# anrieff/fray

Hardware: AMD Instinct MI355X
Metric: Mrays/s (closest-hit + shadow rays) at 1920x1080, 64spp path trace (higher is better)
Workload: dtype f64

## Files before the change

fray_amd/abi.py:

```python
import ctypes as C

i32, u32, i64, u64, f32, f64 = C.c_int32, C.c_uint32, C.c_int64, C.c_uint64, C.c_float, C.c_double
P = C.POINTER

ABI_VERSION = 3

OK, E_ARG, E_PARSE, E_NODEVICE, E_UNSUPPORTED, E_NOMEM, E_HIP, E_CANCELLED = 0, -1, -2, -3, -4, -5, -6, -7
GEOM_PLANE, GEOM_SPHERE, GEOM_CUBE, GEOM_MESH, GEOM_CSG = range(5)
TEX_CHECKER, TEX_BITMAP, TEX_BUMP, TEX_FRESNEL = range(4)
SHADER_CONST, SHADER_LAMBERT, SHADER_PHONG, SHADER_REFL, SHADER_REFR, SHADER_LAYERED = range(6)
LIGHT_POINT, LIGHT_RECT = range(2)
MODE_PRIMARY_ID, MODE_RENDER = 0, 1
FRAME_STATS = 1
OPTION_NAMES = ("pt_lanes", "pt_budget_mib", "speculate_fans", "fused_whitted_max", "fp_contract", "seed_table_mib", "skip_null_segments",
                "segment_planes", "certified_segments")
FIGURE_NAMES = ("contracted_launches", "shadow_segments", "segment_plane_nodes", "certified_segments_eligible", "shadow_segments_certified",
                "shadow_nodes_skipped", "seed_table_bytes", "seed_launches", "seed_planes_reused", "batch_lanes", "whitted_path",
                "pt_budget_effective_mib", "scene_updates", "scene_update_bytes", "arena_bytes", "fans_filed", "fan_children",
                "fan_children_looked_up", "fans_given_up")


class Transform(C.Structure):
    _fields_ = [("offset", f64 * 3), ("m", f64 * 9), ("invM", f64 * 9)]

# ... 256 lines not shown
    "frayhip_unpack_buckets_device": (C.c_int, [VP, VP, C.c_int, C.c_int, C.c_int, C.c_int, C.c_int, VP]),
    "frayhip_bucket_xy": (C.c_int, [C.c_int, C.c_int, C.c_int, C.POINTER(C.c_int), C.POINTER(C.c_int)]),
    "frayhip_comm_available": (C.c_int, []),
    "frayhip_comm_library": (C.c_char_p, []),
    "frayhip_comm_unique_id": (C.c_int, [VP]),
    "frayhip_comm_create": (C.c_int, [VP, C.c_int, C.c_int, P(VP)]),
    "frayhip_comm_from_nccl": (C.c_int, [VP, C.c_int, C.c_int, P(VP)]),
    "frayhip_comm_ranks": (C.c_int, [VP]),
    "frayhip_comm_destroy": (None, [VP]),
    "frayhip_gather_buckets": (C.c_int, [VP, VP, C.c_int, C.c_int, C.c_int, C.c_int, VP]),
    "frayhip_to_rgb32": (C.c_int, [VP, VP, C.c_int]),
    "frayhip_save_bmp": (C.c_int, [C.c_char_p, VP, C.c_int, C.c_int]),
    "frayhip_debug_rng": (C.c_int, [u32, C.c_int, VP, VP, VP, C.c_int]),
    "frayhip_debug_libm": (C.c_int, [C.c_int, VP, VP, VP, VP, VP]),
    "frayhip_debug_arith": (C.c_int, [C.c_int, C.c_int, VP, VP, VP]),
    "frayhip_last_error": (C.c_char_p, []),
    "frayhip_abi_version": (C.c_int, []),
    "frayhip_sizeof": (C.c_int, [C.c_char_p]),
}


def bind(lib):
    for name, (res, args) in SYMBOLS.items():
        fn = getattr(lib, name)
        fn.restype = res
        fn.argtypes = args
    return lib
```

fray_amd/csrc/capi.hip:

```cpp
#include <hip/hip_runtime.h>

#include <algorithm>
#include <chrono>
#include <cstddef>
#include <cmath>
#include <cstring>
#include <string>
#include <vector>
#include <functional>
#include <cstdlib>


#include "entry_support.hpp"
#include "dev_rng.hpp"
#include "dev_pack.hpp"
#include "scene_arena.hpp"

namespace {

using frayhip_detail::set_error;

void put3(double* o, const double* p) { o[0] = p[0]; o[1] = p[1]; o[2] = p[2]; }
}

// ... 292 lines not shown
    std::vector<frayhip_arena::ArenaMeshTables> meshTables;
    std::vector<int64_t> texelOffset;
    std::vector<unsigned char> host;
    std::vector<int64_t> hostOff;
    int32_t counts[11];
    int64_t nTexels;
    std::vector<frayhip_geom_ref> geoms;
    std::vector<frayhip_csg> csgs;
    std::vector<frayhip_mesh> meshes;
    std::vector<frayhip_texture> textures;
    frayhip_environment environment;
};

namespace frayhip_detail {
const DNode* host_nodes(const frayhip_scene* s) { return (const DNode*)(s->edit->host.data() + s->edit->hostOff[s->edit->F.tNodes]); }
}

namespace {

using frayhip_detail::kStatsBytes;
using frayhip_detail::grid_for;

bool create_lanes(frayhip_scene* sc)
{
    if (hipEventCreateWithFlags(&sc->evLaneStart, hipEventDisableTiming) != hipSuccess) return false;
    for (int k = 0; k < FRAY_PT_LANES; k++) {
        if (k > 0 && hipStreamCreateWithFlags(&sc->laneStream[k], hipStreamNonBlocking) != hipSuccess) return false;
        if (hipEventCreateWithFlags(&sc->evResolved[k], hipEventDisableTiming) != hipSuccess) return false;
    }
    return true;
// ... 211 lines not shown
        set_error("frayhip_scene_create: hipMalloc failed (no device?)");
        delete sc;
        return FRAYHIP_E_NODEVICE;
    }
    {
        unsigned char* const base = (unsigned char*)sc->d_arena;
        std::vector<unsigned char*> stage(B.tables.size());
        std::vector<const unsigned char*> addr(B.tables.size());
        for (size_t t = 0; t < B.tables.size(); t++) { stage[t] = B.host.data() + B.tables[t].off; addr[t] = base + B.tables[t].off; }
        frayhip_arena::arena_place(B.F, B.meshTables.data(), B.texelOffset.data(), stage.data(), addr.data(), sc->S);
    }
    hipError_t e = hipMemcpy(sc->d_arena, B.host.data(), B.host.size(), hipMemcpyHostToDevice);
    if (e != hipSuccess) { set_error(std::string("frayhip_scene_create: upload failed: ") + hipGetErrorString(e)); (void)hipFree(sc->d_arena); delete sc; return FRAYHIP_E_NODEVICE; }
    sc->arena_bytes = B.host.size();
    sc->edit = make_scene_edit(d, B);
    sc->camera = d.camera;
    sc->settings = d.settings;
    if (hipMalloc((void**)&sc->d_stats, kStatsBytes) != hipSuccess || hipMalloc((void**)&sc->d_qmeta, 3 * FRAY_PT_LANES * sizeof(QMeta)) != hipSuccess ||
        hipEventCreate(&sc->evA) != hipSuccess || hipEventCreate(&sc->evB) != hipSuccess || !create_lanes(sc)) {
        set_error("frayhip_scene_create: could not allocate the per-scene device state");
        frayhip_scene_destroy(sc);
        return FRAYHIP_E_NOMEM;
    }
    if (const char* e = getenv("FRAYHIP_PT_LANES")) { long v = atol(e); if (v >= 1 && v <= FRAY_PT_LANES) sc->ptLanes = (int)v; }
    if (const char* e = getenv("FRAYHIP_SPECULATE_FANS")) sc->speculateFans = atol(e) != 0;
    if (const char* e = getenv("FRAYHIP_FP_CONTRACT")) sc->fpContract = atol(e) == 1;
    if (const char* e = getenv("FRAYHIP_SKIP_NULL_SEGMENTS")) sc->skipNullSegments = atol(e) != 0;
    if (const char* e = getenv("FRAYHIP_SEGMENT_PLANES")) sc->segmentPlanes = atol(e) != 0;
    if (const char* e = getenv("FRAYHIP_CERTIFIED_SEGMENTS")) sc->certifiedSegments = atol(e) != 0;
    if (const char* e = getenv("FRAYHIP_FUSED_WHITTED_MAX")) { long v = atol(e); if (v >= 0 && v <= 1024) sc->fusedWhittedMax = (int)v; }
// ... 69 lines not shown
        if (value != 0 && value != 1) { set_error("frayhip_scene_set_option: skip_null_segments must be 0 or 1"); return FRAYHIP_E_ARG; }
        s->skipNullSegments = value != 0;
    } else if (n == "segment_planes") {
        if (value != 0 && value != 1) { set_error("frayhip_scene_set_option: segment_planes must be 0 or 1"); return FRAYHIP_E_ARG; }
        s->segmentPlanes = value != 0;
    } else if (n == "certified_segments") {
        if (value != 0 && value != 1) { set_error("frayhip_scene_set_option: certified_segments must be 0 or 1"); return FRAYHIP_E_ARG; }
        s->certifiedSegments = value != 0;
    } else {
        set_error("frayhip_scene_set_option: unknown option " + n);
        return FRAYHIP_E_ARG;
    }
    return FRAYHIP_OK;
}

int frayhip_scene_set_view(frayhip_scene* s, const frayhip_camera* camera, const frayhip_settings* settings)
{
    if (!s) { set_error("frayhip_scene_set_view: null scene"); return FRAYHIP_E_ARG; }
    if (s->rendering) { set_error("frayhip_scene_set_view: the scene is rendering a frame"); return FRAYHIP_E_ARG; }
    if (settings && (settings->frameWidth <= 0 || settings->frameHeight <= 0)) { set_error("frayhip_scene_set_view: bad frame size"); return FRAYHIP_E_ARG; }
    if (camera) s->camera = *camera;
    if (settings) s->settings = *settings;
    return FRAYHIP_OK;
}

int frayhip_scene_update(frayhip_scene* s, const frayhip_scene_desc* desc)
{
    if (!s || !desc) { set_error("frayhip_scene_update: null argument"); return FRAYHIP_E_ARG; }
    if (s->rendering) { set_error("frayhip_scene_update: the scene is rendering a frame"); return FRAYHIP_E_ARG; }
    if (desc->abi_version != FRAYHIP_ABI_VERSION) { set_error("frayhip_scene_update: ABI version mismatch"); return FRAYHIP_E_ARG; }
// ... 16 lines not shown
        addr[t] = (const unsigned char*)s->d_arena + E.tables[t].off;
    }
    frayhip_arena::arena_update(d, E.meshTables.data(), F, tab.data());
    DScene S = s->S;
    frayhip_arena::arena_place(F, E.meshTables.data(), E.texelOffset.data(), tab.data(), addr.data(), S);
    long long bytes = 0;
    for (int32_t t : frayhip_arena::arena_editable_tables(F)) {
        if (!E.tables[t].bytes) continue;
        HIP_TRY(hipMemcpy((unsigned char*)s->d_arena + E.tables[t].off, tab[t], E.tables[t].bytes, hipMemcpyHostToDevice));
        bytes += (long long)E.tables[t].bytes;
    }
    E.host.swap(next);
    E.F = F;
    commit_facts(s, F);
    s->S = S;
    s->sceneUpdates++;
    s->sceneUpdateBytes = bytes;
    return FRAYHIP_OK;
}

void frayhip_scene_destroy(frayhip_scene* s)
{
    if (!s) return;
    delete s->edit;
    if (s->d_arena) (void)hipFree(s->d_arena);
    if (s->d_work) (void)hipFree(s->d_work);
    frayhip_detail::seed_table_free(s);
    if (s->d_stats) (void)hipFree(s->d_stats);
    if (s->d_motionTab) (void)hipFree(s->d_motionTab);
    if (s->d_qmeta) (void)hipFree(s->d_qmeta);
    if (s->evA) (void)hipEventDestroy(s->evA);
    if (s->evB) (void)hipEventDestroy(s->evB);
    if (s->evLaneStart) (void)hipEventDestroy(s->evLaneStart);
    for (int k = 0; k < FRAY_PT_LANES; k++) {
        if (s->evResolved[k]) (void)hipEventDestroy(s->evResolved[k]);
        if (s->laneStream[k]) (void)hipStreamDestroy(s->laneStream[k]);
    }
    for (auto e : s->evPool) (void)hipEventDestroy(e);
    for (auto e : s->evPoolShadow) (void)hipEventDestroy(e);
    delete s;
}
// ... 164 lines not shown
```

fray_amd/csrc/dev_trace.hpp:

```cpp
#pragma once
#ifndef FRAY_IDENTITY_SKIP
#define FRAY_IDENTITY_SKIP 1
#endif
#ifndef FRAY_FILTER_STRAIGHT
#define FRAY_FILTER_STRAIGHT 1
#endif
#include "dev_math.hpp"
#include "dev_scene.hpp"
#include "dev_sort.hpp"
#define FRAY_CERT_SEQ() __builtin_amdgcn_sched_barrier(0)
#include "dev_boxcert.hpp"
#include "dev_misscert.hpp"
#include "dev_segcert.hpp"

#ifdef FRAY_LEAFSTAT
static __device__ unsigned long long g_leafStat[4];
#endif
struct Cnt {
    unsigned long long closest, shadow, node, kdInner, leafRefs, tri, prim, smooth, samples, tex;
    unsigned envelope;
};
template <int ST> FD void bump(unsigned long long& c, unsigned long long n = 1) { if (ST & 1) c += n; }
constexpr bool kd_variant(int st) { return (st & 6) != 0; }
constexpr bool tex_variant(int st) { return (st & 14) != 0; }
// ... 110 lines not shown
        best = gamma;
        l2o = l2;
        l3o = l3;
    }
    return hit;
}

FD void tri_bary(const FRAY_RO DTri* T, V3 s, V3 d, double& l2, double& l3)
{
    const V3 N = ld3(T->N), A = ld3(T->A), AC = ld3(T->AC), AB = ld3(T->AB);
    const V3 D = -d;
    const double rDcr = fray_rcp(dot(N, D));
    const V3 H = s - A;
    l2 = dot(cross(H, AC), D) * rDcr;
    l3 = dot(cross(AB, H), D) * rDcr;
}

FD V3 ray_rdir(V3 d)
{
    V3 rd;
    rd.x = fabs(d.x) > 1e-12 ? fray_rcp(d.x) : 1e12;
    rd.y = fabs(d.y) > 1e-12 ? fray_rcp(d.y) : 1e12;
    rd.z = fabs(d.z) > 1e-12 ? fray_rcp(d.z) : 1e12;
    return rd;
}
template <int ST>
FD void prepare_ray(LocalRay& lr)
{
    if (lr.haveRd) return;
    lr.rd = ray_rdir(lr.d);
// ... 736 lines not shown
        const FRAY_RO DNode& W = S.nodes[best.node];
        if (W.geomKind == 3 && S.meshes[W.geomIndex].smooth) c.smooth++;
    }
    STAMP(6);
    const int nl = S.nLights;
    for (int i = 0; i < nl; i++) {
        double dist;
        if (light_intersect<ST>(S.lights[i], o, d, dist, c) && dist < best.dist) {
            best.node = -2 - i;
            best.dist = dist;
        }
    }
    STAMP(7);
}

FD uint32_t segment_skip_nodes(const DScene& S, V3 a, V3 b, bool live)
{
    const int nP = S.segmentPlanes ? S.nSegPlanes : 0;
    if (nP <= 0) return 0u;
    const V3 e = b - a;
    const double m = seg_cert_scale(a.x, a.y, a.z, b.x, b.y, b.z, e.x, e.y, e.z);
    const lanes_t all = lanes(true);
    uint32_t certified = 0;
    for (int p = 0; p < nP; p++) {
        const FRAY_RO DSegPlane& P = S.segPlanes[p];
        if (lanes(!live || seg_same_side(P.N[0], P.N[1], P.N[2], P.k, P.t0, P.t1, m, a.x, a.y, a.z, b.x, b.y, b.z)) == all) certified |= 1u << p;
    }
    uint32_t skipNodes = 0;
    const int nS = S.nSegNodes;
    for (int j = 0; j < nS; j++)
// ... 77 lines not shown
```

fray_amd/csrc/kernels.hpp:

```cpp
#pragma once
#include "dev_shade.hpp"
#include "dev_whitted.hpp"
#include "dev_queues.hpp"
#include <type_traits>

#ifndef FRAY_PRIMARY_WAVES
#define FRAY_PRIMARY_WAVES 5
#endif
#ifndef FRAY_WHITTED_WAVES
#define FRAY_WHITTED_WAVES 3
#endif
#ifndef FRAY_WHITTED_REFILL
#define FRAY_WHITTED_REFILL 64
#endif
#ifndef FRAY_CSG_WAVES
#define FRAY_CSG_WAVES 3
#endif
constexpr int waves_for(int st, int n) { return (st & 2) ? (FRAY_CSG_WAVES < n ? FRAY_CSG_WAVES : n) : ((st & 1) && n > 2 ? n - 1 : n); }
#ifndef FRAY_MT_EARLY
#define FRAY_MT_EARLY 160
#endif
#ifndef FRAY_WH_SHADE_WAVES
#define FRAY_WH_SHADE_WAVES 4
#endif
// ... 959 lines not shown
        spawn_ray(sh, info, win, ps.tab, wout, brdf, pdf);
        {
            ps.pm = ps.pm * brdf / pdf;
            ps.o = wout.o; ps.d = wout.d; ps.depth = wout.depth; ps.flags = wout.flags;
#ifdef FRAY_SORT_BY_MATERIAL
            ps.flags = (ps.flags & 0xffu) | ((sh.kind == 1 ? 0u : sh.kind == 3 ? 1u : sh.kind == 4 ? 2u : 3u) << 8);
#endif
            if (ps.depth > S.maxTraceDepth || intensity(ps.pm) < 0.01) path_finish(TB, st, ps, SB);
            else cont = true;
        }
    }
    if (!shadow) term_store(TB, ps.slot, own);
}

struct LongRng { uint32_t* cols; uint32_t nPaths; DFrame F; int nItems, s0; };
struct FirstArgs { DCamera C; DFrame F; int nItems, s0; uint32_t n; const uint32_t* x397; unsigned short* termCount; };
struct BounceArgs { DScene S; PathQueue Qin, Qout; ShadowQueue SQ; QMetaRO metaIn; QMeta* metaOut; QMeta* metaShadow; TermBuf TB; StereoBuf SB; LongRng LR; DStats* st; FirstArgs FA; unsigned long long* segCertified; };
#ifndef FRAY_ARITH
#define FRAY_ARITH 0
#endif
template <int ST, bool LONG, bool FIRST = false, int ARITH = FRAY_ARITH>
static __global__ __launch_bounds__(256, waves_for(ST, kd_variant(ST) ? FRAY_BOUNCE_WAVES : FRAY_BOUNCE_WAVES_NOKD)) void k_pt_bounce(BounceArgs A)
{
    static_assert(!(LONG && FIRST), "long generators start from k_pt_init");
    typedef typename std::conditional<LONG, MtPath, Mt>::type G;
    Cnt c = zero_cnt();
    const QMetaRO metaIn = A.metaIn;
    QMeta* const metaOut = A.metaOut;
    QMeta* const metaShadow = A.metaShadow;
    DStats* const st = A.st;
    const FRAY_RO uint32_t* off = FIRST ? nullptr : metaIn.p->off;
    const FRAY_RO uint32_t* nfIn = FIRST ? nullptr : metaIn.p->nf;
    const uint32_t nSeg = FIRST ? 1u : metaIn.p->nSeg, chunkIn = FIRST ? A.FA.n : metaIn.p->chunk;
    const bool certFront = !FIRST && metaIn.p->certFront != 0;
    const WaveShare ws = wave_share(FIRST ? A.FA.n : metaIn.p->n);
    const uint32_t lane = threadIdx.x & 63u;
    SegEnds outEnds{ws.begin, ws.chunk, 0, 0};
    __shared__ uint32_t shadowCount[4][ST == 0 ? 3 : 2];
    if (lane < (ST == 0 ? 3u : 2u)) shadowCount[threadIdx.x >> 6][lane] = 0;
// ... 44 lines not shown
                }
            }
        } else {
            if constexpr (SORT) i = live ? sorted[di - b0] : 0u;
            else i = seg_map(off, nfIn, nSeg, chunkIn, base, di, live, seg);
            gateFree = certFront && (i & FRAY_FRONT_BIT);
            i &= ~FRAY_FRONT_BIT;
            if (live) {
                path_load_ray(Qin, i, ps);
                live = !(ps.d.x == 0 && ps.d.y == 0 && ps.d.z == 0);
            }
        }
        if (live) {
            STAMP(0);
            HitT<ST> h;
            closest_hit<ST>(S, ps.o, ps.d, h, c, gateFree);
            if constexpr (FIRST) {
                ps.pm = c3(1, 1, 1); ps.slot = di; ps.depth = 0; ps.flags = 0;
                ps.rnd = mt_seed_with(seed0, FA.x397[di]);
                ps.tab = ps.rnd;
                mt_skip(ps.rnd, 2);
                if (FA.C.dof) mt_skip(ps.tab, 4);
                bump<ST>(c.samples);
            } else {
                path_load_rest(Qin, i, ps);
            }
#ifdef FRAY_QCHECK
            if (ps.slot >= TB.nPaths) { atomicAdd(&st->rngOverflow, 1ull << 32); ps.slot = 0; ps.pm = c3(0, 0, 0); ps.depth = 0x7fff; }
            else Qin.rec[i].slot = 0xffffffffu;
#endif
            if constexpr (LONG) {
// ... 27 lines not shown
    if (lane == 0) {
        metaOut->cnt[ws.w] = outEnds.nF + outEnds.nB; metaOut->nf[ws.w] = outEnds.nF;
        metaShadow->cnt[ws.w] = shadowCount[threadIdx.x >> 6][0] + shadowCount[threadIdx.x >> 6][1]; metaShadow->nf[ws.w] = shadowCount[threadIdx.x >> 6][0];
        if constexpr (ST == 0) {
            unsigned long long* const total = KARG(BounceArgs, kernel_args<BounceArgs>(), segCertified);
            const uint32_t nCert = shadowCount[threadIdx.x >> 6][2];
            if (total && nCert) atomicAdd(total, (unsigned long long)nCert);
        }
    }
    if (blockIdx.x == 0 && threadIdx.x == 0) {
        metaOut->chunk = ws.chunk; metaOut->nSeg = ws.W; metaShadow->chunk = ws.chunk; metaShadow->nSeg = ws.W;
        metaOut->certFront = metaShadow->certFront = A.S.gatesExact ? 1u : 0u;
    }
    if (ST & 1) flush_stats(st, c);
    if ((ST & 2) && c.envelope) atomicAdd(&st->rngOverflow, 1ull);
}

struct ShadowArgs { DScene S; ShadowQueue SQ; QMetaRO meta; TermBuf TB; DStats* st; unsigned long long* segSkipped; };
template <int ST, int ARITH = FRAY_ARITH>
static __global__ __launch_bounds__(256, anyhit_waves(ST)) void k_pt_shadow(ShadowArgs A)
{
    Cnt c = zero_cnt();
    const QMetaRO meta = A.meta;
    DStats* const st = A.st;
    const FRAY_RO uint32_t* off = meta.p->off;
    const FRAY_RO uint32_t* nfIn = meta.p->nf;
    const uint32_t nSeg = meta.p->nSeg, chunkIn = meta.p->chunk;
    const bool certFront = meta.p->certFront != 0;
    const WaveShare ws = wave_share(meta.p->n);
    const uint32_t lane = threadIdx.x & 63u;
// ... 177 lines not shown
```

fray_amd/csrc/render_impl.hpp:

```cpp
#pragma once
#include <algorithm>
#include <chrono>
#include <cstring>
#include <cstdio>

#include "accum.hpp"
#include "entry_support.hpp"
#include "kernels.hpp"

namespace frayhip_detail {

namespace {
unsigned char* carve_queue(unsigned char* p, size_t n, PathQueue& Q)
{
    Carve c{p};
    Q.rec = (PathRec*)c.take(n * sizeof(PathRec));
    Q.cls = c.take(n);
    return c.p;
}
size_t queue_bytes(size_t n) { return r256(n * sizeof(PathRec)) + r256(n); }
unsigned char* carve_shadow(unsigned char* p, size_t n, ShadowQueue& Q)
{
    Carve c{p};
    Q.ax = (double*)c.take(n * 8); Q.ay = (double*)c.take(n * 8); Q.az = (double*)c.take(n * 8);
// ... 167 lines not shown
    Batches B;
    B.sc = sc; B.prog = prog; B.t0 = t0; B.F = F; B.nItems = nItems; B.d_rgb = d_rgb;
    B.frameBytes = (size_t)W * H * 12;
    B.acc = acc; B.first = first;
    B.total = B.samplesDone = f->mode == FRAYHIP_MODE_PRIMARY_ID ? 1 : first + spp;

    struct Drain { frayhip_scene* sc; bool armed = true; ~Drain() { if (armed) { (void)hipDeviceSynchronize(); seed_table_invalidate(sc); } } } drain{sc};
    sc->seedTab.serving = false;
    sc->lastSeedLaunches = sc->lastSeedReused = 0;
    sc->lastBatchLanes = 1;
    HIP_TRY(hipMemsetAsync(sc->d_stats, 0, kStatsBytes, stream));
    DCursors* cursors = (DCursors*)((unsigned char*)sc->d_stats + kCursorOffset);
    HIP_TRY(hipEventRecord(sc->evA, stream));
    size_t nTraceEvents = 0, nShadowEvents = 0;
    long long nContracted = 0;
    const unsigned long long* fanTotals = nullptr;

    if (f->mode == FRAYHIP_MODE_PRIMARY_ID) {
        if (nItems > 0) {
            hipEvent_t a = pool_event(sc->evPool, 0), b = pool_event(sc->evPool, 1);
            HIP_TRY(hipEventRecord(a, stream));
            hipLaunchKernelGGL(k_primary<ST>, dim3(persistent_grid(nItems, primary_waves(ST))), dim3(256), 0, stream, PrimaryArgs{S, C, F, nItems, d_id, d_dist, sc->d_stats, cursors});
            HIP_TRY(hipEventRecord(b, stream));
            nTraceEvents = 2;
        }
    } else if (f->mode == FRAYHIP_MODE_RENDER) {
        if (!d_rgb && !acc) { set_error("frayhip_render: MODE_RENDER needs an rgb buffer"); return FRAYHIP_E_ARG; }
        if (set.maxTraceDepth < 0) {
            if (nItems > 0 && acc) launch_acc_black(grid_for(nItems), stream, F, nItems, first, spp, sc->camera.stereoSeparation > 0 ? 2 : 1, acc->accum, sc->d_stats);
            else if (nItems > 0) hipLaunchKernelGGL(k_black, dim3(grid_for(nItems)), dim3(256), 0, stream, F, nItems, sc->camera.stereoSeparation > 0 ? 2 : 1, d_rgb, sc->d_stats);
// ... 188 lines not shown
            if (maxLanes > 1 && !(sc->warmMask & warmKey) && !getenv("FRAYHIP_NO_PRIME")) {
                HIP_TRY(hipMemsetAsync(sc->d_qmeta, 0, 3 * FRAY_PT_LANES * sizeof(QMeta), stream));
                HIP_TRY(hipStreamSynchronize(stream));
                for (int k = 0; k < maxLanes; k++) {
                    hipStream_t ws = k == 0 ? stream : sc->laneStream[k];
                    QMeta* m = sc->d_qmeta + 3 * k;
                    const QMetaRO mIn{(const FRAY_RO QMeta*)m};
                    BounceArgs BA{};
                    BA.S = S; BA.metaIn = mIn; BA.metaOut = m + 1; BA.metaShadow = m + 2; BA.st = sc->d_stats;
                    ShadowArgs SA{};
                    SA.S = S; SA.meta = mIn; SA.st = sc->d_stats + 1;
                    if (longRngW) hipLaunchKernelGGL((k_pt_bounce<ST, true>), dim3(1), dim3(256), 0, ws, BA);
                    else {
                        hipLaunchKernelGGL((k_pt_bounce<ST, false>), dim3(1), dim3(256), 0, ws, BA);
                        hipLaunchKernelGGL((k_pt_bounce<ST, false, true>), dim3(1), dim3(256), 0, ws, BA);
                    }
                    hipLaunchKernelGGL(k_pt_shadow<ST>, dim3(1), dim3(256), 0, ws, SA);
                    if constexpr (!(ST & 2)) {
                        if (sc->fpContract) { launch_bounce_contracted<ST>(1, ws, BA); launch_shadow_contracted<ST>(1, ws, SA); }
                    }
                    HIP_TRY(hipStreamSynchronize(ws));
                }
                sc->warmMask |= warmKey;
            }
            if (maxLanes > 3 && (size_t)nItems * (size_t)spp < ((size_t)24 << 20)) maxLanes = 3;
            const bool stereo = sc->camera.stereoSeparation > 0;
            int chunk = 0, nBatches = 0, nLanes = 0;
            size_t nPaths = 0, nQueue = 0, laneBytes = 0;
            if (first == 0) seed_table_begin(sc, F, nItems, spp);
            for (;;) {
// ... 48 lines not shown
                if (!sc->seedTab.serving) { L.seedWords = (uint32_t*)p; p += (nPaths * 4 + 255) / 256 * 256; }
                L.terms = (float*)p; p += (nPaths * (size_t)(set.maxTraceDepth + 2) * 12 + 255) / 256 * 256;
                L.termCount = (unsigned short*)p; p += (nPaths * 2 + 255) / 256 * 256;
                L.mtCols = nullptr;
                if (longRng) { L.mtCols = (uint32_t*)p; p += (nPaths * 2 * 624 * sizeof(uint32_t) + 255) / 256 * 256; }
                L.SB = StereoBuf{};
                L.sampleRadR = nullptr;
                if (stereo) {
                    L.sampleRadR = (float*)p; p += (nPaths * 12 + 255) / 256 * 256;
                    for (int q = 0; q < 6; q++) { L.SB.r[q] = (double*)p; p += (nPaths * 8 + 255) / 256 * 256; }
                    for (int q = 0; q < 6; q++) { L.SB.g[q] = (uint32_t*)p; p += (nPaths * 4 + 255) / 256 * 256; }
                }
            }
            const StereoBuf SBnone{};
            const int nBounce = set.maxTraceDepth + 2;
            HIP_TRY(hipEventRecord(sc->evLaneStart, stream));
            for (int k = 1; k < nLanes; k++) HIP_TRY(hipStreamWaitEvent(sc->laneStream[k], sc->evLaneStart, 0));
            auto trace = [&](int batch) -> int {
                const int s0 = first + batch * chunk, cn = std::min(chunk, spp - batch * chunk);
                Lane& L = lane[batch % nLanes];
                hipStream_t ls = L.stream;
                const uint32_t* x397 = nullptr;
                if (const int rc = seed_batch(sc, F, nItems, s0, cn, L.seedWords, ls, x397)) return rc;
                for (int eye = 0; eye < (stereo ? 2 : 1); eye++) {
                    const bool fused = !stereo && !longRng;
                    float* rad = eye == 0 ? L.sampleRad : L.sampleRadR;
                    const StereoBuf& save = (stereo && eye == 0) ? L.SB : SBnone;
                    if (!fused) {
                        hipLaunchKernelGGL(k_meta_dense, dim3(1), dim3(64), 0, ls, L.meta, (uint32_t)((size_t)nItems * cn));
                        hipLaunchKernelGGL(k_pt_init<ST>, dim3(grid_for((size_t)nItems * cn)), dim3(256), 0, ls, S, C, F, nItems, s0, cn, L.Q[0],
                                           L.termCount, x397, L.SB, eye, sc->d_stats);
                    }
                    for (int b = 0; b < nBounce; b++) {
                        const QMetaRO mIn{(const FRAY_RO QMeta*)(L.meta + (b & 1))}, mSh{(const FRAY_RO QMeta*)(L.meta + 2)};
                        const int grid = bounce_grid((size_t)nItems * cn, (ST & 2) != 0 && nLanes == 1);
                        hipEvent_t ea = pool_event(sc->evPool, nTraceEvents), eb = pool_event(sc->evPool, nTraceEvents + 1);
                        hipEvent_t ec = pool_event(sc->evPoolShadow, nShadowEvents), ed = pool_event(sc->evPoolShadow, nShadowEvents + 1);
                        if (!ea || !eb || !ec || !ed) return FRAYHIP_E_NOMEM;
                        HIP_TRY(hipEventRecord(ea, ls));
                        const LongRng LR{L.mtCols, (uint32_t)nPaths, F, nItems, s0};
                        const TermBuf TB{L.terms, L.termCount, (uint32_t)nPaths, b};
                        const FirstArgs FA{C, F, nItems, s0, (uint32_t)((size_t)nItems * cn), x397, L.termCount};
                        const BounceArgs BA{S, L.Q[b & 1], L.Q[(b + 1) & 1], L.SQ, mIn, L.meta + ((b + 1) & 1), L.meta + 2, TB, save, LR, sc->d_stats, FA, L.segCertified};
                        bool contractedLaunch = false;
                        if constexpr (!(ST & 2)) {
                            if (sc->fpContract && !longRng && b > 0) { launch_bounce_contracted<ST>(grid, ls, BA); contractedLaunch = true; nContracted++; }
                        }
                        if (contractedLaunch) {}
                        else if (longRng) hipLaunchKernelGGL((k_pt_bounce<ST, true>), dim3(grid), dim3(256), 0, ls, BA);
                        else if (fused && b == 0) hipLaunchKernelGGL((k_pt_bounce<ST, false, true>), dim3(grid), dim3(256), 0, ls, BA);
                        else hipLaunchKernelGGL((k_pt_bounce<ST, false>), dim3(grid), dim3(256), 0, ls, BA);
                        HIP_TRY(hipEventRecord(eb, ls));
                        nTraceEvents += 2;
                        hipLaunchKernelGGL(k_scan, dim3(2), dim3(1024), 0, ls, L.meta + ((b + 1) & 1), L.meta + 2, L.segTotal);
                        HIP_TRY(hipEventRecord(ec, ls));
                        bool contractedShadow = false;
                        if constexpr (!(ST & 2)) {
                            if (sc->fpContract) { launch_shadow_contracted<ST>(grid, ls, ShadowArgs{S, L.SQ, mSh, TB, sc->d_stats + 1, L.segSkipped}); contractedShadow = true; nContracted++; }
                        }
                        if (!contractedShadow) hipLaunchKernelGGL(k_pt_shadow<ST>, dim3(grid), dim3(256), 0, ls, ShadowArgs{S, L.SQ, mSh, TB, sc->d_stats + 1, L.segSkipped});
                        HIP_TRY(hipEventRecord(ed, ls));
                        nShadowEvents += 2;
                    }
                    if (stereo) hipLaunchKernelGGL(k_pt_fold, dim3(grid_for((size_t)nItems * cn)), dim3(256), 0, ls, TermBuf{L.terms, L.termCount, (uint32_t)nPaths, 0},
// ... 31 lines not shown
                  "the shadow-queue totals, the skipped nodes and the certified segments follow the counter blocks");
    HIP_TRY(hipMemcpy(&back, sc->d_stats, sizeof back, hipMemcpyDeviceToHost));
    const DStats (&dsv)[2] = back.ds;
    sc->lastShadowSegments = 0;
    for (int k = 0; k < FRAY_PT_LANES; k++) sc->lastShadowSegments += (long long)back.segTotal[k];
    sc->lastShadowCertified = 0;
    for (int k = 0; k < FRAY_PT_LANES; k++) sc->lastShadowCertified += (long long)back.segCertified[k];
    sc->lastShadowSegments += sc->lastShadowCertified;
    sc->lastShadowNodesSkipped = 0;
    for (int k = 0; k < FRAY_PT_LANES; k++) sc->lastShadowNodesSkipped += (long long)back.segSkipped[k];
    {
        unsigned long long ft[4] = {0, 0, 0, 0};
        if (fanTotals) HIP_TRY(hipMemcpy(ft, fanTotals, sizeof ft, hipMemcpyDeviceToHost));
        for (int q = 0; q < 4; q++) sc->lastFans[q] = (long long)ft[q];
        sc->lastContracted = nContracted;
    }
#ifdef FRAY_LEAFSTAT
    {
        unsigned long long ls[4] = {0, 0, 0, 0}, zero[4] = {0, 0, 0, 0};
        (void)hipMemcpyFromSymbol(ls, HIP_SYMBOL(g_leafStat), sizeof ls);
        (void)hipMemcpyToSymbol(HIP_SYMBOL(g_leafStat), zero, sizeof zero);
        if (ls[0]) fprintf(stderr, "[leafstat] wave leaf phases %llu, all active lanes in ONE leaf %.1f %%, active lanes per phase %.1f, distinct leaves per phase %.2f\n",
                           ls[0], 100.0 * (double)ls[1] / (double)ls[0], (double)ls[2] / (double)ls[0], (double)ls[3] / (double)ls[0]);
    }
#endif
#ifdef FRAY_TILESTAT
    if (const char* out = getenv("FRAY_TILESTAT_OUT")) {
        std::vector<unsigned long long> ts(65536 * 8);
        (void)hipMemcpyFromSymbol(ts.data(), HIP_SYMBOL(g_tileStat), ts.size() * sizeof(unsigned long long));
        if (FILE* fp = fopen(out, "wb")) { fwrite(ts.data(), sizeof(unsigned long long), ts.size(), fp); fclose(fp); }
// ... 51 lines not shown
```

fray_amd/csrc/render_state.hpp:

```cpp
#pragma once
#include <hip/hip_runtime.h>

#include <cstddef>
#include <string>
#include <vector>

#include "capi_common.h"
#include "dev_scene.hpp"
#include "dev_queues.hpp"

namespace frayhip_detail {
inline int hip_error_code(hipError_t e)
{
    switch (e) {
        case hipErrorOutOfMemory: return FRAYHIP_E_NOMEM;
        case hipErrorNoDevice: case hipErrorInvalidDevice: case hipErrorInsufficientDriver: case hipErrorNotInitialized: return FRAYHIP_E_NODEVICE;
        default: return FRAYHIP_E_HIP;
    }
}
}
#define HIP_TRY(expr)                                                                             \
    do {                                                                                          \
        hipError_t e_ = (expr);                                                                   \
        if (e_ != hipSuccess) {                                                                   \
// ... 35 lines not shown
    frayhip_camera camera{};
    frayhip_settings settings{};
    bool whittedNeedsRecursion = false;
    int specFanMax = 0;
    bool speculateFans = true;
    bool lightDraws = false;
    int lastWhittedPath = 0;
    int fusedWhittedMax = 4;
    int csgLanes = 1;
    unsigned warmMask = 0;
    bool fpContract = false;
    long long lastContracted = 0;
    bool skipNullSegments = true;
    bool segmentPlanes = true;
    bool certifiedSegments = true;
    long long lastShadowCertified = 0;
    long long lastShadowNodesSkipped = 0;
    long long lastShadowSegments = 0;
    long long lastFans[4] = {0, 0, 0, 0};
    int lightSampleCount = 0;
    bool extGeometry = false;
    bool textured = false;
    bool kdMeshes = false;
    void* d_work = nullptr;
    size_t work_bytes = 0;
    DStats* d_stats = nullptr;
    void* d_motionTab = nullptr;
    size_t motionTabBytes = 0;
    std::vector<unsigned char> motionTabHost;
    QMeta* d_qmeta = nullptr;
// ... 43 lines not shown
```

fray_amd/scene.py:

```python
import ctypes as C
import math
import os
import sys

import numpy as np

from . import abi

P = C.POINTER

_HERE = os.path.dirname(os.path.abspath(__file__))
_LIB_PATH = os.environ.get("FRAYHIP_LIB") or os.path.join(_HERE, "libfrayhip.so")


class FrayError(RuntimeError):
    def __init__(self, code, msg):
        super().__init__("frayhip error %d: %s" % (code, msg))
        self.code = code


def _load():
    if "torch" not in sys.modules and not os.environ.get("FRAYHIP_NO_TORCH"):
        try:
            import torch
# ... 545 lines not shown
    def endRender(self):
        if self._dev:
            lib.frayhip_scene_destroy(self._dev)
            self._dev = C.c_void_p()

    def set_option(self, name, value):
        self._need_dev()
        _check(lib.frayhip_scene_set_option(self._dev, name.encode(), int(value)))
        return self

    def get_option(self, name):
        self._need_dev()
        v = C.c_int64(0)
        _check(lib.frayhip_scene_get_option(self._dev, name.encode(), C.byref(v)))
        return int(v.value)

    def _frame(self, mode, seed, bucket_first, bucket_stride, spp_chunk, stats):
        return abi.Frame(mode=mode, seed=seed, bucket_first=bucket_first, bucket_stride=bucket_stride,
                         spp_chunk=spp_chunk, flags=abi.FRAME_STATS if stats else 0)

    def _need_dev(self):
        if not self._dev:
            raise FrayError(abi.E_ARG, "Scene.beginRender() has not been called")

    def render(self, seed=42, bucket_first=0, bucket_stride=1, spp_chunk=0, stats=False, out=None, progress=None, preview_ms=-1):
        self._need_dev()
        W, H = self.frame_size
        rgb = out if out is not None else np.zeros((H, W, 3), np.float32)
        st = abi.Stats()
        fr = self._frame(abi.MODE_RENDER, seed, bucket_first, bucket_stride, spp_chunk, stats)
# ... 514 lines not shown
```

include/frayhip.h:

```cpp
#ifndef FRAYHIP_H
#define FRAYHIP_H

#include <stdint.h>

#ifdef __cplusplus
extern "C" {
#endif

#define FRAYHIP_ABI_VERSION 3

enum {
    FRAYHIP_OK            = 0,
    FRAYHIP_E_ARG         = -1,
    FRAYHIP_E_PARSE       = -2,
    FRAYHIP_E_NODEVICE    = -3,
    FRAYHIP_E_UNSUPPORTED = -4,
    FRAYHIP_E_NOMEM       = -5,
    FRAYHIP_E_HIP         = -6,
    FRAYHIP_E_CANCELLED   = -7,
};


typedef struct frayhip_transform {
    double offset[3];
// ... 397 lines not shown
int  frayhip_comm_unique_id(void* id128);
int  frayhip_comm_create(const void* id128, int rank, int world, frayhip_comm** out);
int  frayhip_comm_from_nccl(void* nccl_comm, int rank, int world, frayhip_comm** out);
int  frayhip_comm_ranks(frayhip_comm* c);
void frayhip_comm_destroy(frayhip_comm* c);
int  frayhip_gather_buckets(frayhip_comm* c, float* d_frame, int width, int height, int channels, int root, void* hip_stream);

int  frayhip_to_rgb32(const float* rgb, uint32_t* out, int n_pixels);

int  frayhip_save_bmp(const char* path, const float* rgb, int width, int height);

int  frayhip_debug_rng(uint32_t seed, int n, float* floats, double* doubles, int32_t* ints, int int_hi);

int  frayhip_debug_libm(int n, const double* x, double* sin_out, double* cos_out, double* acos_out, double* acos_arg);

int  frayhip_debug_arith(int op, int n, const double* a, const double* b, double* out);

const char* frayhip_last_error(void);
int  frayhip_abi_version(void);
int  frayhip_sizeof(const char* struct_name);

#ifdef __cplusplus
}
#endif
#endif
```

Baseline: 13290.

## Precompute per-frame camera-origin table for first-bounce triangle tests

Adds a per-frame kernel that, for the camera position, precomputes each node's local-space origin and per-triangle origin-dependent terms (N·H, H×AC, AB×H). The fused first-bounce kernel then uses a specialised closest-hit that reads these values instead of recomputing the transform and cross products per ray. This cuts arithmetic for primary rays in exchange for extra memory traffic, a small single-block setup kernel, and a device buffer sized by the triangle count. It is enabled by default for the plain stats-free path and skipped for stereo, depth of field and long RNG.

```diff
diff --git a/fray_amd/abi.py b/fray_amd/abi.py
--- a/fray_amd/abi.py
+++ b/fray_amd/abi.py
@@ -294,6 +294,7 @@
     "frayhip_debug_rng": (C.c_int, [u32, C.c_int, VP, VP, VP, C.c_int]),
     "frayhip_debug_libm": (C.c_int, [C.c_int, VP, VP, VP, VP, VP]),
     "frayhip_debug_arith": (C.c_int, [C.c_int, C.c_int, VP, VP, VP]),
+    "frayhip_debug_camera_table": (C.c_int, [VP, P(C.c_int64)]),
     "frayhip_last_error": (C.c_char_p, []),
     "frayhip_abi_version": (C.c_int, []),
     "frayhip_sizeof": (C.c_int, [C.c_char_p]),
diff --git a/fray_amd/csrc/capi.hip b/fray_amd/csrc/capi.hip
--- a/fray_amd/csrc/capi.hip
+++ b/fray_amd/csrc/capi.hip
@@ -330,6 +330,13 @@
 
 namespace frayhip_detail {
 const DNode* host_nodes(const frayhip_scene* s) { return (const DNode*)(s->edit->host.data() + s->edit->hostOff[s->edit->F.tNodes]); }
+int count_tl_tris(const frayhip_scene* s)
+{
+    const DNode* nodes = host_nodes(s);
+    long long n = 0;
+    for (int i = 0; i < s->edit->F.nNodes; i++) n += nodes[i].tlTris;
+    return (int)std::min<long long>(n, 0x7fffffff);
+}
 }
 
 namespace {
@@ -571,6 +578,7 @@
     if (e != hipSuccess) { set_error(std::string("frayhip_scene_create: upload failed: ") + hipGetErrorString(e)); (void)hipFree(sc->d_arena); delete sc; return FRAYHIP_E_NODEVICE; }
     sc->arena_bytes = B.host.size();
     sc->edit = make_scene_edit(d, B);
+    sc->camTabTris = frayhip_detail::count_tl_tris(sc);
     sc->camera = d.camera;
     sc->settings = d.settings;
     if (hipMalloc((void**)&sc->d_stats, kStatsBytes) != hipSuccess || hipMalloc((void**)&sc->d_qmeta, 3 * FRAY_PT_LANES * sizeof(QMeta)) != hipSuccess ||
@@ -670,6 +678,13 @@
     return FRAYHIP_OK;
 }
 
+int frayhip_debug_camera_table(frayhip_scene* s, int64_t* used)
+{
+    if (!s || !used) { set_error("frayhip_debug_camera_table: null argument"); return FRAYHIP_E_ARG; }
+    *used = s->lastCameraTable ? 1 : 0;
+    return FRAYHIP_OK;
+}
+
 int frayhip_scene_set_view(frayhip_scene* s, const frayhip_camera* camera, const frayhip_settings* settings)
 {
     if (!s) { set_error("frayhip_scene_set_view: null scene"); return FRAYHIP_E_ARG; }
@@ -716,6 +731,7 @@
     E.F = F;
     commit_facts(s, F);
     s->S = S;
+    s->camTabTris = frayhip_detail::count_tl_tris(s);
     s->sceneUpdates++;
     s->sceneUpdateBytes = bytes;
     return FRAYHIP_OK;
@@ -727,6 +743,7 @@
     delete s->edit;
     if (s->d_arena) (void)hipFree(s->d_arena);
     if (s->d_work) (void)hipFree(s->d_work);
+    if (s->d_camTab) (void)hipFree(s->d_camTab);
     frayhip_detail::seed_table_free(s);
     if (s->d_stats) (void)hipFree(s->d_stats);
     if (s->d_motionTab) (void)hipFree(s->d_motionTab);
diff --git a/fray_amd/csrc/dev_trace.hpp b/fray_amd/csrc/dev_trace.hpp
--- a/fray_amd/csrc/dev_trace.hpp
+++ b/fray_amd/csrc/dev_trace.hpp
@@ -148,6 +148,48 @@
     const V3 H = s - A;
     l2 = dot(cross(H, AC), D) * rDcr;
     l3 = dot(cross(AB, H), D) * rDcr;
+}
+
+struct CamNode { double s[3]; int32_t zero, triBase; };
+struct CamTri { double NH, HAC[3], ABH[3], pad; };
+struct CamTab { const FRAY_RO CamNode* nodes; const FRAY_RO CamTri* tris; };
+FD V3 cam_local_origin(const FRAY_RO DNode& N, V3 o) { return mulM(o - ld3(N.T.off), N.T.inv); }
+FD void cam_tri_fill(const FRAY_RO DTri* T, V3 s, double& NH, V3& HAC, V3& ABH)
+{
+    const V3 N = ld3(T->N), A = ld3(T->A), AC = ld3(T->AC), AB = ld3(T->AB);
+    V3 H = s - A;
+    NH = dot(N, H);
+    HAC = cross(H, AC);
+    ABH = cross(AB, H);
+}
+template <int ST>
+FD bool tri_test_cam(const FRAY_RO DTri* T, const FRAY_RO CamTri* R, int culling, V3 d, double& best, double& l2o, double& l3o, Cnt& c)
+{
+    bump<ST>(c.tri);
+    const V3 g = ld3(T->g), N = ld3(T->N);
+    lanes_t ok = lanes(!(dot(d, g) > 0));
+    if (!culling) ok = lanes(true);
+    V3 D = -d;
+    double Dcr = dot(N, D);
+    ok &= lanes(!(fabs(Dcr) < 1e-12));
+    if (!ok) return false;
+    double rDcr = fray_rcp(Dcr);
+    double gamma = R->NH * rDcr;
+    ok &= lanes(!(gamma < 0)) & lanes(!(gamma > best));
+    if (!ok) return false;
+    double l2 = dot(ld3(R->HAC), D) * rDcr;
+    ok &= lanes(!(l2 < 0)) & lanes(!(l2 > 1));
+    double l3 = dot(ld3(R->ABH), D) * rDcr;
+    ok &= lanes(!(l3 < 0)) & lanes(!(l3 > 1));
+    double l1 = 1 - (l2 + l3);
+    ok &= lanes(!(l1 < 0));
+    const bool hit = lane_of(ok);
+    if (hit) {
+        best = gamma;
+        l2o = l2;
+        l3o = l3;
+    }
+    return hit;
 }
 
 FD V3 ray_rdir(V3 d)
@@ -914,6 +956,85 @@
     STAMP(7);
 }
 
+template <int ST>
+FD bool node_intersect_cam(const DScene& S, int i, V3 o, V3 d, LocalRay& lr, double& dist, double& t, int& tri, double& l2, double& l3, Cnt& c, const CamTab& cam)
+{
+    static_assert(ST == 0 && FRAY_ARITH == 0, "the camera table serves flag word 0 in the exact arithmetic");
+    bump<ST>(c.node);
+    const FRAY_RO DNode& N = S.nodes[i];
+    const FRAY_RO CamNode& K = cam.nodes[i];
+    if (N.xfClass != lr.cls) {
+        const bool zeros = d.x == 0 || d.y == 0 || d.z == 0;
+        if (N.xfIdentity && !K.zero && !__any(zeros)) lr.d = normalized(d);
+        else lr.d = normalized(mulM(d, N.T.inv));
+        lr.s = ld3(K.s);
+        lr.cls = N.xfClass;
+        lr.haveRd = false;
+    }
+    STAMP(1);
+    V3 ipl;
+    if (N.tlTris > 0) {
+        prepare_ray<ST>(lr);
+        const V3 ls = lr.s, ld = lr.d;
+        Box6 box;
+        box.lox = N.bmin[0]; box.loy = N.bmin[1]; box.loz = N.bmin[2];
+        box.hix = N.bmax[0]; box.hiy = N.bmax[1]; box.hiz = N.bmax[2];
+        const FRAY_RO DNodeX& X = S.nodesX[i];
+        Box6 be;
+        be.lox = X.bminE[0]; be.loy = X.bminE[1]; be.loz = X.bminE[2];
+        be.hix = X.bmaxE[0]; be.hiy = X.bmaxE[1]; be.hiz = X.bmaxE[2];
+        const bool rootHit = box_test_pre(box, be, ls, ld, lr.rd);
+        STAMP(2);
+        if (!rootHit) return false;
+        double gamma = 1e99;
+        bool found = false;
+        const int n = N.tlTris, culling = N.tlCulling;
+        const FRAY_RO DTri* tris = N.tlPtr;
+        const FRAY_RO CamTri* R = cam.tris + K.triBase;
+        for (int k = 0; k < n; k++)
+            if (tri_test_cam<ST>(tris + k, R + k, culling, ld, gamma, l2, l3, c)) { found = true; tri = k; }
+        STAMP(3);
+        if (!found) return false;
+        ipl = ls + ld * gamma;
+        t = gamma;
+    } else if (!geom_intersect<ST>(S, N, i, lr, ipl, t, tri, l2, l3, nullptr, c)) return false;
+    STAMP(5);
+    const V3 ipw = N.xfIdentity ? ipl : mulM(ipl, N.T.m) + ld3(N.T.off);
+    dist = length(o - ipw);
+    STAMP(6);
+    return true;
+}
+template <int ST>
+FD void closest_hit_cam(const DScene& S, V3 o, V3 d, HitT<ST>& best, Cnt& c, const CamTab& cam)
+{
+    bump<ST>(c.closest);
+    best.node = -1;
+    best.tri = -1;
+    best.dist = 1e99;
+    best.t = 0; best.l2 = 0; best.l3 = 0;
+    const int nn = S.nNodes;
+    LocalRay lr;
+    lr.cls = -1;
+    lr.haveRd = false;
+    for (int i = 0; i < nn; i++) {
+        double dist, t, l2 = 0, l3 = 0;
+        int tri = -1;
+        if (node_intersect_cam<ST>(S, i, o, d, lr, dist, t, tri, l2, l3, c, cam) && dist < best.dist) {
+            best.node = i; best.tri = tri; best.dist = dist; best.t = t; best.l2 = l2; best.l3 = l3;
+        }
+    }
+    STAMP(6);
+    const int nl = S.nLights;
+    for (int i = 0; i < nl; i++) {
+        double dist;
+        if (light_intersect<ST>(S.lights[i], o, d, dist, c) && dist < best.dist) {
+            best.node = -2 - i;
+            best.dist = dist;
+        }
+    }
+    STAMP(7);
+}
+
 FD uint32_t segment_skip_nodes(const DScene& S, V3 a, V3 b, bool live)
 {
     const int nP = S.segmentPlanes ? S.nSegPlanes : 0;
diff --git a/fray_amd/csrc/kernels.hpp b/fray_amd/csrc/kernels.hpp
--- a/fray_amd/csrc/kernels.hpp
+++ b/fray_amd/csrc/kernels.hpp
@@ -997,15 +997,16 @@
 }
 
 struct LongRng { uint32_t* cols; uint32_t nPaths; DFrame F; int nItems, s0; };
-struct FirstArgs { DCamera C; DFrame F; int nItems, s0; uint32_t n; const uint32_t* x397; unsigned short* termCount; };
+struct FirstArgs { DCamera C; DFrame F; int nItems, s0; uint32_t n; const uint32_t* x397; unsigned short* termCount; CamTab cam; };
 struct BounceArgs { DScene S; PathQueue Qin, Qout; ShadowQueue SQ; QMetaRO metaIn; QMeta* metaOut; QMeta* metaShadow; TermBuf TB; StereoBuf SB; LongRng LR; DStats* st; FirstArgs FA; unsigned long long* segCertified; };
 #ifndef FRAY_ARITH
 #define FRAY_ARITH 0
 #endif
-template <int ST, bool LONG, bool FIRST = false, int ARITH = FRAY_ARITH>
+template <int ST, bool LONG, bool FIRST = false, int ARITH = FRAY_ARITH, bool CAM = false>
 static __global__ __launch_bounds__(256, waves_for(ST, kd_variant(ST) ? FRAY_BOUNCE_WAVES : FRAY_BOUNCE_WAVES_NOKD)) void k_pt_bounce(BounceArgs A)
 {
     static_assert(!(LONG && FIRST), "long generators start from k_pt_init");
+    static_assert(!CAM || (FIRST && ST == 0 && ARITH == 0), "the camera table serves the fused first bounce of flag word 0");
     typedef typename std::conditional<LONG, MtPath, Mt>::type G;
     Cnt c = zero_cnt();
     const QMetaRO metaIn = A.metaIn;
@@ -1080,7 +1081,8 @@
         if (live) {
             STAMP(0);
             HitT<ST> h;
-            closest_hit<ST>(S, ps.o, ps.d, h, c, gateFree);
+            if constexpr (CAM) closest_hit_cam<ST>(S, ps.o, ps.d, h, c, FA.cam);
+            else closest_hit<ST>(S, ps.o, ps.d, h, c, gateFree);
             if constexpr (FIRST) {
                 ps.pm = c3(1, 1, 1); ps.slot = di; ps.depth = 0; ps.flags = 0;
                 ps.rnd = mt_seed_with(seed0, FA.x397[di]);
@@ -1138,6 +1140,37 @@
     }
     if (ST & 1) flush_stats(st, c);
     if ((ST & 2) && c.envelope) atomicAdd(&st->rngOverflow, 1ull);
+}
+
+static __global__ __launch_bounds__(256) void k_camera_table(DScene S, double ox, double oy, double oz, CamNode* __restrict__ nodes, CamTri* __restrict__ tris)
+{
+    const V3 o = v3(ox, oy, oz);
+    const int nn = S.nNodes;
+    for (int i = (int)threadIdx.x; i < nn; i += (int)blockDim.x) {
+        const V3 s = cam_local_origin(S.nodes[i], o);
+        nodes[i].s[0] = s.x; nodes[i].s[1] = s.y; nodes[i].s[2] = s.z;
+        nodes[i].zero = (o.x == 0 || o.y == 0 || o.z == 0) ? 1 : 0;
+    }
+    if (threadIdx.x == 0) {
+        int base = 0;
+        for (int i = 0; i < nn; i++) { nodes[i].triBase = base; base += S.nodes[i].tlTris; }
+    }
+    __syncthreads();
+    for (int i = 0; i < nn; i++) {
+        const int n = S.nodes[i].tlTris;
+        if (n <= 0) continue;
+        const V3 s = v3(nodes[i].s[0], nodes[i].s[1], nodes[i].s[2]);
+        CamTri* const R = tris + nodes[i].triBase;
+        for (int t = (int)threadIdx.x; t < n; t += (int)blockDim.x) {
+            double NH;
+            V3 HAC, ABH;
+            cam_tri_fill(S.nodes[i].tlPtr + t, s, NH, HAC, ABH);
+            R[t].NH = NH;
+            R[t].HAC[0] = HAC.x; R[t].HAC[1] = HAC.y; R[t].HAC[2] = HAC.z;
+            R[t].ABH[0] = ABH.x; R[t].ABH[1] = ABH.y; R[t].ABH[2] = ABH.z;
+            R[t].pad = 0;
+        }
+    }
 }
 
 struct ShadowArgs { DScene S; ShadowQueue SQ; QMetaRO meta; TermBuf TB; DStats* st; unsigned long long* segSkipped; };
diff --git a/fray_amd/csrc/render_impl.hpp b/fray_amd/csrc/render_impl.hpp
--- a/fray_amd/csrc/render_impl.hpp
+++ b/fray_amd/csrc/render_impl.hpp
@@ -205,6 +205,7 @@
     HIP_TRY(hipEventRecord(sc->evA, stream));
     size_t nTraceEvents = 0, nShadowEvents = 0;
     long long nContracted = 0;
+    bool camTabUsed = false;
     const unsigned long long* fanTotals = nullptr;
 
     if (f->mode == FRAYHIP_MODE_PRIMARY_ID) {
@@ -423,6 +424,7 @@
                     else {
                         hipLaunchKernelGGL((k_pt_bounce<ST, false>), dim3(1), dim3(256), 0, ws, BA);
                         hipLaunchKernelGGL((k_pt_bounce<ST, false, true>), dim3(1), dim3(256), 0, ws, BA);
+                        if constexpr (ST == 0) hipLaunchKernelGGL((k_pt_bounce<ST, false, true, FRAY_ARITH, true>), dim3(1), dim3(256), 0, ws, BA);
                     }
                     hipLaunchKernelGGL(k_pt_shadow<ST>, dim3(1), dim3(256), 0, ws, SA);
                     if constexpr (!(ST & 2)) {
@@ -501,6 +503,25 @@
             }
             const StereoBuf SBnone{};
             const int nBounce = set.maxTraceDepth + 2;
+            CamTab camTab{};
+            if constexpr (ST == 0) {
+                const char* const camEnv = getenv("FRAYHIP_CAMERA_TABLE");
+                if (!(camEnv && atol(camEnv) == 0) && !stereo && !longRng && !C.dof && S.nNodes > 0) {
+                    const size_t need = (size_t)S.nNodes * sizeof(CamNode) + (size_t)sc->camTabTris * sizeof(CamTri);
+                    if (need > sc->camTabBytes) {
+                        if (sc->d_camTab) (void)hipFree(sc->d_camTab);
+                        sc->d_camTab = nullptr; sc->camTabBytes = 0;
+                        if (hipMalloc(&sc->d_camTab, need) == hipSuccess) sc->camTabBytes = need; else { sc->d_camTab = nullptr; (void)hipGetLastError(); }
+                    }
+                    if (sc->d_camTab) {
+                        CamNode* const cn = (CamNode*)sc->d_camTab;
+                        CamTri* const ct = (CamTri*)(cn + S.nNodes);
+                        hipLaunchKernelGGL(k_camera_table, dim3(1), dim3(256), 0, stream, S, C.pos[0], C.pos[1], C.pos[2], cn, ct);
+                        camTab.nodes = (const FRAY_RO CamNode*)cn; camTab.tris = (const FRAY_RO CamTri*)ct;
+                        camTabUsed = true;
+                    }
+                }
+            }
             HIP_TRY(hipEventRecord(sc->evLaneStart, stream));
             for (int k = 1; k < nLanes; k++) HIP_TRY(hipStreamWaitEvent(sc->laneStream[k], sc->evLaneStart, 0));
             auto trace = [&](int batch) -> int {
@@ -527,7 +548,7 @@
                         HIP_TRY(hipEventRecord(ea, ls));
                         const LongRng LR{L.mtCols, (uint32_t)nPaths, F, nItems, s0};
                         const TermBuf TB{L.terms, L.termCount, (uint32_t)nPaths, b};
-                        const FirstArgs FA{C, F, nItems, s0, (uint32_t)((size_t)nItems * cn), x397, L.termCount};
+                        const FirstArgs FA{C, F, nItems, s0, (uint32_t)((size_t)nItems * cn), x397, L.termCount, camTab};
                         const BounceArgs BA{S, L.Q[b & 1], L.Q[(b + 1) & 1], L.SQ, mIn, L.meta + ((b + 1) & 1), L.meta + 2, TB, save, LR, sc->d_stats, FA, L.segCertified};
                         bool contractedLaunch = false;
                         if constexpr (!(ST & 2)) {
@@ -535,6 +556,7 @@
                         }
                         if (contractedLaunch) {}
                         else if (longRng) hipLaunchKernelGGL((k_pt_bounce<ST, true>), dim3(grid), dim3(256), 0, ls, BA);
+                        else if (fused && b == 0 && camTabUsed) { if constexpr (ST == 0) hipLaunchKernelGGL((k_pt_bounce<ST, false, true, FRAY_ARITH, true>), dim3(grid), dim3(256), 0, ls, BA); }
                         else if (fused && b == 0) hipLaunchKernelGGL((k_pt_bounce<ST, false, true>), dim3(grid), dim3(256), 0, ls, BA);
                         else hipLaunchKernelGGL((k_pt_bounce<ST, false>), dim3(grid), dim3(256), 0, ls, BA);
                         HIP_TRY(hipEventRecord(eb, ls));
@@ -596,6 +618,7 @@
         if (fanTotals) HIP_TRY(hipMemcpy(ft, fanTotals, sizeof ft, hipMemcpyDeviceToHost));
         for (int q = 0; q < 4; q++) sc->lastFans[q] = (long long)ft[q];
         sc->lastContracted = nContracted;
+        sc->lastCameraTable = camTabUsed;
     }
 #ifdef FRAY_LEAFSTAT
     {
diff --git a/fray_amd/csrc/render_state.hpp b/fray_amd/csrc/render_state.hpp
--- a/fray_amd/csrc/render_state.hpp
+++ b/fray_amd/csrc/render_state.hpp
@@ -73,6 +73,10 @@
     bool skipNullSegments = true;
     bool segmentPlanes = true;
     bool certifiedSegments = true;
+    bool lastCameraTable = false;
+    int camTabTris = 0;
+    void* d_camTab = nullptr;
+    size_t camTabBytes = 0;
     long long lastShadowCertified = 0;
     long long lastShadowNodesSkipped = 0;
     long long lastShadowSegments = 0;
diff --git a/fray_amd/scene.py b/fray_amd/scene.py
--- a/fray_amd/scene.py
+++ b/fray_amd/scene.py
@@ -583,6 +583,12 @@
         v = C.c_int64(0)
         _check(lib.frayhip_scene_get_option(self._dev, name.encode(), C.byref(v)))
         return int(v.value)
+
+    def camera_table_used(self):
+        self._need_dev()
+        v = C.c_int64(0)
+        _check(lib.frayhip_debug_camera_table(self._dev, C.byref(v)))
+        return bool(v.value)
 
     def _frame(self, mode, seed, bucket_first, bucket_stride, spp_chunk, stats):
         return abi.Frame(mode=mode, seed=seed, bucket_first=bucket_first, bucket_stride=bucket_stride,
diff --git a/include/frayhip.h b/include/frayhip.h
--- a/include/frayhip.h
+++ b/include/frayhip.h
@@ -435,6 +435,7 @@
 
 int  frayhip_debug_libm(int n, const double* x, double* sin_out, double* cos_out, double* acos_out, double* acos_arg);
 
+int  frayhip_debug_camera_table(frayhip_scene* s, int64_t* used);
 int  frayhip_debug_arith(int op, int n, const double* a, const double* b, double* out);
 
 const char* frayhip_last_error(void);
```

After: 13400, median of 5. Within noise of the previous version (+0.8%).
